# scientificcomputing/networks_fenicsx

Measured on NVIDIA B200. Metric: tree-network assemble+solve DOFs/s, higher is better.
Workload: dtype f64

## Files before the change

### networks_fenicsx_b200/_build.py

```python

from __future__ import annotations

import os
import pathlib
import shutil
import subprocess

CSRC = pathlib.Path(__file__).parent / "csrc"
LIB = CSRC / "libnxfx_b200.so"
SOURCES = ["nxfx_b200.cu"]
HEADERS = ["ctx.cuh", "assemble.cuh", "spmv.cuh", "precond.cuh", "generic.cuh", "condense.cuh", "peer.cuh", "../../include/nxfx_b200.h"]


def nvcc_path() -> str:
    for cand in (os.environ.get("NVCC"), shutil.which("nvcc"), "/usr/local/cuda/bin/nvcc"):
        if cand and os.path.exists(cand):
            return cand
    raise RuntimeError("nvcc not found; libnxfx_b200.so cannot be built")


def is_stale() -> bool:
    if not LIB.exists():
        return True
    t = LIB.stat().st_mtime
    return any((CSRC / f).resolve().stat().st_mtime > t for f in SOURCES + HEADERS)


def build_library(force: bool = False, verbose: bool = False) -> pathlib.Path:
    if not force and not is_stale():
        return LIB
    cmd = [
        nvcc_path(),
        "-gencode", "arch=compute_100a,code=sm_100a",
        "-O3", "-lineinfo", "-std=c++17",
        "-Xcompiler", "-fPIC", "-shared",
        "-o", str(LIB),
    ] + [str(CSRC / s) for s in SOURCES]
    if verbose:
        cmd.insert(1, "-Xptxas=-v")
    proc = subprocess.run(cmd, capture_output=True, text=True)
    if proc.returncode != 0:
        raise RuntimeError(f"nvcc failed:\n{' '.join(cmd)}\n{proc.stdout}\n{proc.stderr}")
    if verbose:
        print(proc.stderr)
    return LIB
```

### networks_fenicsx_b200/csrc/assemble.cuh

```cuda
#pragma once

#include "ctx.cuh"

namespace nxfx {

struct FastDiv {
  uint32_t magic, shift;
};
inline FastDiv make_fastdiv(uint32_t d) {
  FastDiv f;
  uint32_t fl = 31;
  while (!((d >> fl) & 1u)) --fl;
  if ((d & (d - 1)) == 0) {
    f.magic = 0;
    f.shift = fl == 0 ? 0 : fl - 1;
  } else {
    const uint64_t n = 1ull << (32 + fl);
    uint64_t m = n / d;
    const uint64_t rem = n % d;
    m += m;
    if (2 * rem >= d) m += 1;
    f.magic = (uint32_t)(m + 1);
    f.shift = fl;
  }
  return f;
}
__device__ __forceinline__ int fastdiv(int n, FastDiv f) {
  const uint32_t t = __umulhi((uint32_t)n, f.magic);
  return (int)(((((uint32_t)n - t) >> 1) + t) >> f.shift);
}

struct Net {
  int32_t n_nodes, E, N, n_bif;
  int32_t nq, poff, loff, ndofs;
  FastDiv div_np1, div_n;
  const int4* __restrict__ slot_uvl;
  const int32_t* __restrict__ slot_edge;
  const int32_t* __restrict__ edge_slot;
  const int32_t* __restrict__ bif_ptr;
  const int32_t* __restrict__ bif_inc;
  const double2* __restrict__ x2;
  const int2* __restrict__ slot_uv;
  const uint32_t* __restrict__ bif_in_bits;
};

constexpr unsigned int kLmTag = 0x7FF8B1F0u;
__device__ __forceinline__ double lm_box(int lm) {
  return __hiloint2double((int)kLmTag, lm);
}
__device__ __forceinline__ int lm_unbox(double p) {
  return (unsigned int)__double2hiint(p) == kLmTag ? __double2loint(p) : -1;
}

struct Coef {
  const double* __restrict__ R_cell;
  const double* __restrict__ f_cell;
  double R_const, f_const;
  double* __restrict__ cell_rh;
};

constexpr double kThird = 1.0 / 3.0;
constexpr double kSixth = 1.0 / 6.0;
constexpr int kMaxFluxRow = 7;

__device__ __forceinline__ int vertex_id(const Net& g, int e, int u, int v, int a) {
  return a == 0 ? u : (a == g.N ? v : g.n_nodes + e * (g.N - 1) + (a - 1));
}

struct VertexRec {
  double x, y, z, p;
};

__device__ __forceinline__ VertexRec load_vertex(const double2* __restrict__ x2, int v) {
  const double2* p = x2 + 2 * (size_t)v;
  const double2 a = __ldg(p), b = __ldg(p + 1);
  return VertexRec{a.x, a.y, b.x, b.y};
}

__device__ __forceinline__ double seg_length(const VertexRec& v0, const VertexRec& v1) {
  const double dx = __dsub_rn(v1.x, v0.x), dy = __dsub_rn(v1.y, v0.y), dz = __dsub_rn(v1.z, v0.z);
  return __dsqrt_rn(
      __dadd_rn(__dadd_rn(__dmul_rn(dx, dx), __dmul_rn(dy, dy)), __dmul_rn(dz, dz)));
}

__global__ void __launch_bounds__(kThreads)
pad_nodes_kernel(int n_nodes, int gdim, const double* __restrict__ pos, double* __restrict__ x) {
  int i = blockIdx.x * blockDim.x + threadIdx.x;
  if (i >= n_nodes * 3) return;
  int node = i / 3, d = i - node * 3;
  x[4 * (size_t)node + d] = d < gdim ? pos[(size_t)node * gdim + d] : 0.0;
}

__global__ void __launch_bounds__(kThreads)
set_pbc_kernel(int64_t nv, const double* __restrict__ pbc, double* __restrict__ x) {
  const int64_t i = blockIdx.x * (int64_t)blockDim.x + threadIdx.x;
  if (i < nv && lm_unbox(x[4 * i + 3]) < 0) x[4 * i + 3] = pbc[i];
}

__global__ void __launch_bounds__(kThreads)
tag_lm_kernel(int n_nodes, const int32_t* __restrict__ node_lm, double* __restrict__ x) {
  const int i = blockIdx.x * blockDim.x + threadIdx.x;
  if (i < n_nodes && node_lm[i] >= 0) x[4 * (size_t)i + 3] = lm_box(node_lm[i]);
}

__global__ void __launch_bounds__(kThreads)
interior_vertices_kernel(int n_nodes, int E, int N, const int32_t* __restrict__ eu,
                         const int32_t* __restrict__ ev, double* __restrict__ x) {
  const int64_t total = (int64_t)E * (N - 1) * 3;
  const double step = 1.0 / (double)N;
  for (int64_t i = blockIdx.x * (int64_t)blockDim.x + threadIdx.x; i < total;
       i += (int64_t)gridDim.x * blockDim.x) {
    const int64_t vert = i / 3;
    const int d = (int)(i - vert * 3);
    const int e = (int)(vert / (N - 1));
    const int k = (int)(vert - (int64_t)e * (N - 1)) + 1;
    const double w = __dmul_rn((double)k, step);
    const double s = x[4 * (size_t)eu[e] + d], t = x[4 * (size_t)ev[e] + d];
    x[4 * ((size_t)n_nodes + vert) + d] = __dadd_rn(__dmul_rn(s, __dsub_rn(1.0, w)), __dmul_rn(t, w));
  }
}

__device__ __forceinline__ int flux_row_cols(const Net& g, int r, int* cols) {
  const int N = g.N, np1 = N + 1;
  const int slot = r / np1, a = r - slot * np1;
  const int4 t = g.slot_uvl[slot];
  const int e = g.slot_edge[slot];
// ... 393 lines not shown
```

### networks_fenicsx_b200/csrc/ctx.cuh

```cuda
#pragma once

#include <cuda_runtime.h>

#include <cstdarg>
#include <cstdint>
#include <cstdio>
#include <cstring>
#include <string>
#include <vector>

#include "../../include/nxfx_b200.h"

namespace nxfx {

constexpr int kTileRows = 256;
constexpr int kTileCap = 2048;
constexpr int kThreads = 256;

template <typename T>
struct DevBuf {
  T* p = nullptr;
  size_t n = 0;
  cudaError_t alloc(size_t count) {
    release();
    n = count;
    if (count == 0) return cudaSuccess;
    return cudaMalloc(reinterpret_cast<void**>(&p), count * sizeof(T));
  }
  void release() {
    if (p) cudaFree(p);
    p = nullptr;
    n = 0;
  }
  ~DevBuf() { release(); }
};

struct TreeSchedule {
  bool set = false;
  int n_chunks = 0, n_lvl_ptr = 0, n_chords = 0, n_top = 0;
  int top_b0 = 0;
  std::vector<int32_t> t_of_bif_h;
  std::vector<int32_t> top_lvl_h;
  int sh_lmax = -1, pr_lmin = 0;
  int cap = 2048;
  DevBuf<int32_t> bif_of_t, chunk_desc, t_inc_ptr;
  DevBuf<int2> t_inc;
  DevBuf<double> lam_nat;
  DevBuf<int32_t> t_of_bif, t_parent, t_pedge, t_pslot, t_cptr, t_cidx, chunk_lptr, lvl_ptr, chord_edge;
  DevBuf<double> diag0, tg, d, gd, r, lam;
  bool fast_ok = false;
  bool coop_ok = false;
  bool coop_fs_ok = false;
  int coop_fs_blocks = 0;
  unsigned int epoch = 0;
};

struct MatState {
  int64_t id = 0;
  DevBuf<double> vals;
  DevBuf<double> cell_rh;
  bool assembled = false;
  int acc_count = 0;
};

struct Condensation {
  bool set = false;
  int n_max = 0, kl = 0, per_edge = 0, pcell_base = 0, pcell_stride = 0, cont = 0;
  DevBuf<int32_t> type_n, loc_ptr, loc_kind, loc_off, k_ptr, k_row, k_col, k_cell, c_ptr, c_row, c_slot, d_ptr, d_slot,
      d_col, bif_node, ipiv;
  DevBuf<double> k_coef, c_coef, d_coef, band, Y, S, y0, h, bd0, bU, bL, bDinv, bG, bH, br, bz;
  std::vector<int32_t> bif_node_h;
};

struct PeerComm {
  bool created = false, ready = false;
  bool in_process = false;
  bool shared_device = false;
  int rank = 0, nranks = 1;
  int slot = 0;
  void* local = nullptr;
  void* base[16] = {};
  unsigned int epoch[2] = {0, 0};
  int* err_h = nullptr;
  int* err_d = nullptr;
  DevBuf<double> lam_scratch;
};

}

struct nxfx_ctx {
  int device = 0;
  cudaStream_t stream = nullptr;
  std::string err;
  int64_t launches = 0;
  cudaEvent_t ev0 = nullptr, ev1 = nullptr;
  int sm_count = 148;

  bool has_network = false, has_pattern = false, has_pbc = false, pc_ready = false;
  bool bottom_factored = false;
  int32_t n_nodes = 0, E = 0, gdim = 0, N = 0, n_bif = 0, n_inc = 0;
  int64_t nv = 0, nc = 0, nq = 0, poff = 0, loff = 0, ndofs = 0, nnz = 0;
  nxfx::DevBuf<double> x;
  nxfx::DevBuf<double> pos_stage;
  nxfx::DevBuf<int4> slot_uvl;
  nxfx::DevBuf<int2> slot_uv;
  nxfx::DevBuf<uint32_t> bif_in_bits;
  nxfx::DevBuf<int32_t> slot_edge, edge_slot, edge_u, edge_v, bif_ptr, bif_inc;
  nxfx::DevBuf<int32_t> rowptr, colidx, tile_base;
  bool pipe_ok = false;
  bool generic = false;
  nxfx::DevBuf<int32_t> gen_src_id, gen_bptr, gen_bid;
  nxfx::DevBuf<double> gen_src_coef, gen_bcoef, gen_cell_h;
  nxfx::Condensation cond;
  std::vector<nxfx::MatState*> mats;
  nxfx::MatState* cur = nullptr;
  int64_t next_mat_id = 1;
  bool pc_unscaled = false;
  int64_t pc_mat = -1;
  std::vector<int32_t> edge_slot_h;
  nxfx::TreeSchedule tree;
  nxfx::DevBuf<double> edge_g, edge_c, edge_fn;
  nxfx::DevBuf<double> work;
  nxfx::DevBuf<double> work2;
  nxfx::DevBuf<double> scal;
  nxfx::DevBuf<unsigned int> ticket;
  double* scal_h = nullptr;
  double* scal_h_dev = nullptr;
  bool pdl_coop_refused = false;
  int32_t n_shared = 0;
  nxfx::DevBuf<int32_t> shared_lm;
  std::vector<int32_t> shared_lm_h;
  nxfx::DevBuf<int32_t> top_sh_pos;
  nxfx::DevBuf<int32_t> top_sh_idx;
  nxfx::DevBuf<double> lam_weight, lam_nonshared;
  nxfx::DevBuf<double> p_nonshared;
  nxfx::PeerComm comm;
  uint64_t peer_on = 0;
  double* mirror_h = nullptr;
  cudaStream_t side = nullptr;
  cudaEvent_t ev_x = nullptr;
  nxfx::DevBuf<double> e2e_pbc, e2e_b, e2e_x;
};

namespace nxfx {

inline int fail(nxfx_ctx* ctx, int code, const char* fmt, ...) {
  char buf[512];
  va_list ap;
  va_start(ap, fmt);
  vsnprintf(buf, sizeof buf, fmt, ap);
  va_end(ap);
  if (ctx) ctx->err = buf;
  return code;
}

#define NXFX_CUDA(ctx, call)                                                                  \
  do {                                                                                        \
    cudaError_t _e = (call);                                                                  \
    if (_e != cudaSuccess)                                                                    \
      return nxfx::fail(ctx, NXFX_ERR_CUDA, "%s:%d: %s -> %s", __FILE__, __LINE__, #call,     \
                        cudaGetErrorString(_e));                                              \
  } while (0)

#define NXFX_REQUIRE(ctx, cond, msg)                                                          \
  do {                                                                                        \
    if (!(cond)) return nxfx::fail(ctx, NXFX_ERR_INVALID, "%s: %s", __func__, msg);           \
  } while (0)

#define NXFX_LAUNCH(ctx, kernel, grid, block, smem, ...)                                      \
  do {                                                                                        \
    kernel<<<(grid), (block), (smem), (ctx)->stream>>>(__VA_ARGS__);                          \
    (ctx)->launches++;                                                                        \
    NXFX_CUDA(ctx, cudaGetLastError());                                                       \
  } while (0)

inline int64_t cdiv(int64_t a, int64_t b) { return (a + b - 1) / b; }

}
```

### networks_fenicsx_b200/csrc/nxfx_b200.cu

```cuda

#include <cub/device/device_scan.cuh>

#include <algorithm>
#include <atomic>
#include <chrono>
#include <cmath>
#include <cstdlib>

#include "assemble.cuh"
#include "ctx.cuh"
#include "condense.cuh"
#include "generic.cuh"
#include "precond.cuh"
#include "spmv.cuh"

using namespace nxfx;

namespace {

constexpr int kScalPartials = 8 * kMaxPartials;
constexpr int kScalSlots = 1024;

Net make_net(const nxfx_ctx* c) {
  Net g;
  g.n_nodes = c->n_nodes;
  g.E = c->E;
  g.N = c->N;
  g.n_bif = c->n_bif;
  g.nq = (int32_t)c->nq;
  g.poff = (int32_t)c->poff;
  g.loff = (int32_t)c->loff;
  g.ndofs = (int32_t)c->ndofs;
  g.div_np1 = make_fastdiv((uint32_t)c->N + 1);
  g.div_n = make_fastdiv((uint32_t)std::max(c->N, 2));
  g.slot_uvl = c->slot_uvl.p;
  g.slot_edge = c->slot_edge.p;
  g.edge_slot = c->edge_slot.p;
  g.bif_ptr = c->bif_ptr.p;
  g.bif_inc = c->bif_inc.p;
  g.x2 = reinterpret_cast<const double2*>(c->x.p);
  g.slot_uv = c->slot_uv.p;
  g.bif_in_bits = c->bif_in_bits.p;
  return g;
}

TreeDev make_tree(nxfx_ctx* c) {
  TreeDev t;
  auto& s = c->tree;
  t.t_of_bif = s.t_of_bif.p;
  t.bif_of_t = s.bif_of_t.p;
  t.chunk_desc = s.chunk_desc.p;
  t.t_inc_ptr = s.t_inc_ptr.p;
  t.t_inc = s.t_inc.p;
  t.lam_nat = s.lam_nat.p;
  t.cap = s.cap;
  t.top_sh_pos = c->top_sh_pos.p;
  t.n_sh = c->top_sh_pos.p ? c->n_shared : 0;
  t.sh_lmax = s.sh_lmax;
  t.pr_lmin = s.pr_lmin;
  t.t_parent = s.t_parent.p;
  t.t_pedge = s.t_pedge.p;
  t.t_pslot = s.t_pslot.p;
  t.t_cptr = s.t_cptr.p;
  t.t_cidx = s.t_cidx.p;
  t.chunk_lptr = s.chunk_lptr.p;
  t.lvl_ptr = s.lvl_ptr.p;
  t.diag0 = s.diag0.p;
  t.tg = s.tg.p;
  t.d = s.d.p;
  t.gd = s.gd.p;
  t.r = s.r.p;
  t.lam = s.lam.p;
  return t;
}

PeerDev make_peer(nxfx_ctx* c, int ch) {
  PeerDev p = {};
  if (!c->comm.ready) return p;
  for (int r = 0; r < c->comm.nranks; ++r) p.base[r] = reinterpret_cast<unsigned long long>(c->comm.base[r]);
  p.rank = c->comm.rank;
  p.nranks = c->comm.nranks;
  p.slot = c->comm.slot;
  p.epoch = ++c->comm.epoch[ch];
  p.err = c->comm.err_d;
  return p;
}

CondDev make_cond(nxfx_ctx* ctx) {
  auto& k = ctx->cond;
  CondDev c;
  c.n_max = k.n_max; c.kl = k.kl; c.kv = 2 * k.kl; c.ldab = 3 * k.kl + 1;
  c.per_edge = k.per_edge; c.pcell_base = k.pcell_base; c.pcell_stride = k.pcell_stride; c.cont = k.cont;
  c.type_n = k.type_n.p; c.loc_ptr = k.loc_ptr.p; c.loc_kind = k.loc_kind.p; c.loc_off = k.loc_off.p;
  c.k_ptr = k.k_ptr.p; c.k_row = k.k_row.p; c.k_col = k.k_col.p; c.k_cell = k.k_cell.p; c.k_coef = k.k_coef.p;
  c.c_ptr = k.c_ptr.p; c.c_row = k.c_row.p; c.c_slot = k.c_slot.p; c.c_coef = k.c_coef.p;
  c.d_ptr = k.d_ptr.p; c.d_slot = k.d_slot.p; c.d_col = k.d_col.p; c.d_coef = k.d_coef.p;
  c.bif_node = k.bif_node.p;
  c.band = k.band.p; c.ipiv = k.ipiv.p; c.Y = k.Y.p; c.S = k.S.p; c.y0 = k.y0.p; c.h = k.h.p;
  c.bd0 = k.bd0.p; c.bU = k.bU.p; c.bL = k.bL.p; c.bDinv = k.bDinv.p; c.bG = k.bG.p; c.bH = k.bH.p;
  c.br = k.br.p; c.bz = k.bz.p;
  return c;
}

int vec_grid(const nxfx_ctx* c, int64_t n) {
  return (int)std::max<int64_t>(1, std::min<int64_t>(cdiv(n, kThreads), (int64_t)c->sm_count * 8));
}

template <typename T>
int upload(nxfx_ctx* ctx, DevBuf<T>& buf, const T* src, size_t n) {
  NXFX_CUDA(ctx, buf.alloc(n));
  if (n) NXFX_CUDA(ctx, cudaMemcpyAsync(buf.p, src, n * sizeof(T), cudaMemcpyHostToDevice, ctx->stream));
  return NXFX_OK;
}

int update_top_shared(nxfx_ctx* ctx) {
  ctx->top_sh_pos.release();
  ctx->top_sh_idx.release();
  ctx->tree.sh_lmax = -1;
  ctx->tree.pr_lmin = 0;
  if (!ctx->tree.set || ctx->n_shared == 0 || ctx->tree.t_of_bif_h.empty()) return NXFX_OK;
  std::vector<int32_t> pos((size_t)ctx->n_shared);
  for (int32_t i = 0; i < ctx->n_shared; ++i) {
    const int32_t p = ctx->tree.t_of_bif_h[ctx->shared_lm_h[i]] - ctx->tree.top_b0;
    if (p < 0 || p >= ctx->tree.n_top)
      return fail(ctx, NXFX_ERR_INVALID, "shared multiplier %d is not in the top chunk of the schedule", ctx->shared_lm_h[i]);
// ... 46 lines not shown

void release_matrices(nxfx_ctx* ctx) {
  for (MatState* m : ctx->mats) delete m;
  ctx->mats.clear();
  ctx->cur = nullptr;
  ctx->pc_ready = false;
  ctx->pc_mat = -1;
}

int new_matrix(nxfx_ctx* ctx, int64_t id, MatState** out) {
  auto* m = new MatState();
  m->id = id;
  ctx->mats.push_back(m);
  NXFX_CUDA(ctx, m->vals.alloc((size_t)ctx->nnz + 8));
  NXFX_CUDA(ctx, cudaMemsetAsync(m->vals.p, 0, ((size_t)ctx->nnz + 8) * sizeof(double), ctx->stream));
  NXFX_CUDA(ctx, m->cell_rh.alloc((size_t)ctx->nc));
  NXFX_CUDA(ctx, cudaMemsetAsync(m->cell_rh.p, 0, (size_t)ctx->nc * sizeof(double), ctx->stream));
  if (out) *out = m;
  return NXFX_OK;
}

void note_lhs_assembled(nxfx_ctx* ctx, int accumulate) {
  MatState* m = ctx->cur;
  m->acc_count = (accumulate && m->assembled) ? m->acc_count + 1 : 1;
  m->assembled = true;
  ctx->pc_ready = false;
  ctx->bottom_factored = false;
}

void bind_matrix(nxfx_ctx* ctx, MatState* m) {
  if (ctx->cur != m) ctx->bottom_factored = false;
  ctx->cur = m;
  if (ctx->pc_ready && ctx->pc_mat != m->id) ctx->pc_ready = false;
}

void mark_factored(nxfx_ctx* ctx) {
  ctx->pc_ready = true;
  ctx->pc_mat = ctx->cur->id;
}

int ensure_matrix(nxfx_ctx* ctx) {
  if (ctx->cur) return NXFX_OK;
  for (MatState* m : ctx->mats)
    if (m->id == 0) { bind_matrix(ctx, m); return NXFX_OK; }
  MatState* m = nullptr;
  int rc = new_matrix(ctx, 0, &m);
  if (rc) return rc;
  bind_matrix(ctx, m);
  return NXFX_OK;
}

int build_vertices(nxfx_ctx* ctx) {
  const int n3 = ctx->n_nodes * 3;
  NXFX_LAUNCH(ctx, pad_nodes_kernel, (int)cdiv(n3, kThreads), kThreads, 0, ctx->n_nodes, ctx->gdim,
              ctx->pos_stage.p, ctx->x.p);
  if (ctx->N > 1) {
    const int64_t total = (int64_t)ctx->E * (ctx->N - 1) * 3;
    NXFX_LAUNCH(ctx, interior_vertices_kernel, vec_grid(ctx, total), kThreads, 0, ctx->n_nodes,
                ctx->E, ctx->N, ctx->edge_u.p, ctx->edge_v.p, ctx->x.p);
  }
  return NXFX_OK;
}

constexpr size_t kPipeSmem = kStages * sizeof(SpmvStage) + kStages * sizeof(uint64_t);
#ifndef NXFX_SPMV_BLOCKS
#define NXFX_SPMV_BLOCKS 5
#endif
constexpr int kPipeBlocksPerSM = NXFX_SPMV_BLOCKS;

int do_spmv(nxfx_ctx* ctx, const double* x, double* y) {
  const int ntiles = (int)cdiv(ctx->ndofs, kTileRows);
  if (ctx->pipe_ok) {
    const int grid = std::min(ntiles, ctx->sm_count * kPipeBlocksPerSM);
    NXFX_LAUNCH(ctx, spmv_pipe_kernel<0>, grid, kTileRows, kPipeSmem, (int)ctx->ndofs, ntiles,
                ctx->rowptr.p, ctx->colidx.p, ctx->cur->vals.p, ctx->tile_base.p, x, y, nullptr, nullptr,
                nullptr, nullptr);
    return NXFX_OK;
  }
  NXFX_LAUNCH(ctx, spmv_kernel<0>, ntiles, kTileRows, 0, (int)ctx->ndofs, ntiles, ctx->rowptr.p,
              ctx->colidx.p, ctx->cur->vals.p, x, y, nullptr, nullptr, nullptr, nullptr);
  return NXFX_OK;
}

int do_residual(nxfx_ctx* ctx, const double* b, const double* x, double* r, double* norm2_d, bool pdl = false) {
  const int ntiles = (int)cdiv(ctx->ndofs, kTileRows);
  if (ctx->comm.ready) {
    NXFX_REQUIRE(ctx, ctx->pipe_ok && ctx->lam_nonshared.p, "the fused partitioned residual needs the pipelined SpMV and nxfx_set_shared");
    const int grid = std::min(ntiles, ctx->sm_count * kPipeBlocksPerSM);
    cudaLaunchConfig_t cfg = {};
    cfg.gridDim = dim3(grid);
    cfg.blockDim = dim3(kTileRows);
    cfg.dynamicSmemBytes = kPipeSmem;
    cfg.stream = ctx->stream;
    cudaLaunchAttribute attr[1];
    attr[0].id = cudaLaunchAttributeProgrammaticStreamSerialization;
    attr[0].val.programmaticStreamSerializationAllowed = 1;
    cfg.attrs = attr;
    cfg.numAttrs = pdl ? 1 : 0;
    NXFX_CUDA(ctx, cudaLaunchKernelEx(&cfg, spmv_pipe_kernel<3>, (int)ctx->ndofs, ntiles, (const int32_t*)ctx->rowptr.p,
                                      (const int32_t*)ctx->colidx.p, (const double*)ctx->cur->vals.p,
                                      (const int32_t*)ctx->tile_base.p, x, r, b, ctx->scal.p, ctx->ticket.p, norm2_d,
                                      (int)ctx->loff, (const double*)ctx->lam_nonshared.p, (const double*)ctx->lam_weight.p,
                                      make_peer(ctx, 1), (const int32_t*)ctx->shared_lm.p, (int)ctx->n_shared,
                                      ctx->comm.lam_scratch.p));
    ctx->launches++;
    return NXFX_OK;
  }
  if (ctx->pipe_ok && !pdl) {
    const int grid = std::min(ntiles, ctx->sm_count * kPipeBlocksPerSM);
    NXFX_LAUNCH(ctx, spmv_pipe_kernel<1>, grid, kTileRows, kPipeSmem, (int)ctx->ndofs, ntiles,
                ctx->rowptr.p, ctx->colidx.p, ctx->cur->vals.p, ctx->tile_base.p, x, r, b, ctx->scal.p,
                ctx->ticket.p, norm2_d);
    return NXFX_OK;
  }
  if (ctx->pipe_ok) {
    const int grid = std::min(ntiles, ctx->sm_count * kPipeBlocksPerSM);
    cudaLaunchConfig_t cfg = {};
    cfg.gridDim = dim3(grid);
    cfg.blockDim = dim3(kTileRows);
    cfg.dynamicSmemBytes = kPipeSmem;
    cfg.stream = ctx->stream;
    cudaLaunchAttribute attr[1];
    attr[0].id = cudaLaunchAttributeProgrammaticStreamSerialization;
    attr[0].val.programmaticStreamSerializationAllowed = 1;
    cfg.attrs = attr;
    cfg.numAttrs = 1;
    NXFX_CUDA(ctx, cudaLaunchKernelEx(&cfg, spmv_pipe_kernel<1>, (int)ctx->ndofs, ntiles, (const int32_t*)ctx->rowptr.p,
                                      (const int32_t*)ctx->colidx.p, (const double*)ctx->cur->vals.p,
                                      (const int32_t*)ctx->tile_base.p, x, r, b, ctx->scal.p, ctx->ticket.p, norm2_d, 0,
                                      (const double*)nullptr, (const double*)nullptr, PeerDev{}, (const int32_t*)nullptr, 0,
                                      (double*)nullptr));
    ctx->launches++;
    return NXFX_OK;
  }
  const int grid = std::min(ntiles, kMaxPartials);
  NXFX_LAUNCH(ctx, spmv_kernel<1>, grid, kTileRows, 0, (int)ctx->ndofs, ntiles, ctx->rowptr.p,
              ctx->colidx.p, ctx->cur->vals.p, x, r, b, ctx->scal.p, ctx->ticket.p, norm2_d);
  return NXFX_OK;
}

template <int K>
int launch_multi_dot(nxfx_ctx* ctx, int n, const double* A, size_t stride, const double* w, double* out) {
  NXFX_LAUNCH(ctx, multi_dot_kernel<K>, vec_grid(ctx, n), kThreads, 0, n, A, stride, w, ctx->scal.p,
              ctx->ticket.p, out);
  return NXFX_OK;
}

int do_multi_dot(nxfx_ctx* ctx, int n, int k, const double* A, size_t stride, const double* w, double* out) {
  int j = 0;
  while (j < k) {
    const int m = std::min(8, k - j);
    const double* Aj = A + (size_t)j * stride;
    int rc = NXFX_OK;
    switch (m) {
      case 8: rc = launch_multi_dot<8>(ctx, n, Aj, stride, w, out + j); break;
      case 7: rc = launch_multi_dot<7>(ctx, n, Aj, stride, w, out + j); break;
      case 6: rc = launch_multi_dot<6>(ctx, n, Aj, stride, w, out + j); break;
      case 5: rc = launch_multi_dot<5>(ctx, n, Aj, stride, w, out + j); break;
      case 4: rc = launch_multi_dot<4>(ctx, n, Aj, stride, w, out + j); break;
      case 3: rc = launch_multi_dot<3>(ctx, n, Aj, stride, w, out + j); break;
      case 2: rc = launch_multi_dot<2>(ctx, n, Aj, stride, w, out + j); break;
      default: rc = launch_multi_dot<1>(ctx, n, Aj, stride, w, out + j); break;
    }
    if (rc) return rc;
    j += m;
  }
  return NXFX_OK;
// ... 669 lines not shown
  if (!ctx) return NXFX_ERR_INVALID;
  NXFX_CUDA(ctx, cudaMemcpyAsync(d, s, bytes, cudaMemcpyDeviceToHost, ctx->stream));
  return NXFX_OK;
}
int nxfx_memcpy_d2d(nxfx_ctx* ctx, void* d, const void* s, size_t bytes) {
  if (!ctx) return NXFX_ERR_INVALID;
  NXFX_CUDA(ctx, cudaMemcpyAsync(d, s, bytes, cudaMemcpyDeviceToDevice, ctx->stream));
  return NXFX_OK;
}
int nxfx_memset(nxfx_ctx* ctx, void* d, int byte, size_t bytes) {
  if (!ctx) return NXFX_ERR_INVALID;
  NXFX_CUDA(ctx, cudaMemsetAsync(d, byte, bytes, ctx->stream));
  return NXFX_OK;
}
int nxfx_timer_start(nxfx_ctx* ctx) {
  if (!ctx) return NXFX_ERR_INVALID;
  NXFX_CUDA(ctx, cudaEventRecord(ctx->ev0, ctx->stream));
  return NXFX_OK;
}
int nxfx_timer_stop(nxfx_ctx* ctx, double* ms) {
  if (!ctx || !ms) return NXFX_ERR_INVALID;
  NXFX_CUDA(ctx, cudaEventRecord(ctx->ev1, ctx->stream));
  NXFX_CUDA(ctx, cudaEventSynchronize(ctx->ev1));
  float f = 0.f;
  NXFX_CUDA(ctx, cudaEventElapsedTime(&f, ctx->ev0, ctx->ev1));
  *ms = f;
  return NXFX_OK;
}

int nxfx_set_network(nxfx_ctx* ctx, int32_t n_nodes, int32_t n_edges, int32_t gdim, int32_t N,
                     const double* node_pos, const int32_t* edge_u, const int32_t* edge_v,
                     const int32_t* edge_slot, const int32_t* node_lm, int32_t n_bif,
                     const int32_t* bif_ptr, const int32_t* bif_inc) {
  if (!ctx) return NXFX_ERR_INVALID;
  NXFX_REQUIRE(ctx, n_nodes > 0 && n_edges > 0 && N >= 1 && gdim >= 1 && gdim <= 3, "bad sizes");
  NXFX_REQUIRE(ctx, node_pos && edge_u && edge_v && edge_slot && node_lm && bif_ptr, "null input");
  NXFX_CUDA(ctx, cudaSetDevice(ctx->device));
  const int64_t E = n_edges;
  const int64_t nq = E * (N + 1), nc = E * N, ndofs = nq + nc + n_bif;
  const int64_t nv = (int64_t)n_nodes + E * (N - 1);
  NXFX_REQUIRE(ctx, ndofs < (int64_t)2147483000 && nv * 3 < (int64_t)2147483000, "network too large for int32 indexing");
  const int32_t n_inc = bif_ptr[n_bif];
  NXFX_REQUIRE(ctx, n_inc == 0 || bif_inc, "null incidence list");
  std::vector<int4> uvl((size_t)E);
  std::vector<int32_t> slot_edge((size_t)E, -1);
  for (int64_t e = 0; e < E; ++e) {
    const int32_t u = edge_u[e], v = edge_v[e], s = edge_slot[e];
    if (u < 0 || u >= n_nodes || v < 0 || v >= n_nodes || u == v)
      return fail(ctx, NXFX_ERR_INVALID, "edge %lld has invalid endpoints (%d, %d)", (long long)e, u, v);
    if (s < 0 || s >= E || slot_edge[s] != -1)
      return fail(ctx, NXFX_ERR_INVALID, "edge_slot is not a permutation (edge %lld -> %d)", (long long)e, s);
    if (node_lm[u] >= n_bif || node_lm[v] >= n_bif)
      return fail(ctx, NXFX_ERR_INVALID, "node_lm out of range at edge %lld", (long long)e);
    slot_edge[s] = (int32_t)e;
    uvl[s] = make_int4(u, v, node_lm[u], node_lm[v]);
  }
  for (int32_t k = 0; k < n_inc; ++k)
    if ((bif_inc[k] >> 1) < 0 || (bif_inc[k] >> 1) >= E)
      return fail(ctx, NXFX_ERR_INVALID, "bif_inc[%d] out of range", k);
  ctx->has_network = ctx->has_pattern = ctx->has_pbc = ctx->pc_ready = false;
  release_matrices(ctx);
  nxfx_comm_destroy(ctx);
  ctx->edge_slot_h.assign(edge_slot, edge_slot + E);
  ctx->n_shared = 0;
  ctx->shared_lm.release();
  ctx->shared_lm_h.clear();
  ctx->top_sh_pos.release();
  ctx->top_sh_idx.release();
  ctx->tree.t_of_bif_h.clear();
  ctx->lam_weight.release();
  ctx->lam_nonshared.release();
  ctx->p_nonshared.release();
  ctx->tree.set = false;
  ctx->n_nodes = n_nodes; ctx->E = n_edges; ctx->gdim = gdim; ctx->N = N; ctx->n_bif = n_bif;
  ctx->n_inc = n_inc; ctx->nv = nv; ctx->nc = nc; ctx->nq = nq; ctx->poff = nq; ctx->loff = nq + nc;
  ctx->ndofs = ndofs; ctx->nnz = 0;
  int rc;
  if ((rc = upload(ctx, ctx->pos_stage, node_pos, (size_t)n_nodes * gdim))) return rc;
  if ((rc = upload(ctx, ctx->edge_u, edge_u, (size_t)E))) return rc;
  if ((rc = upload(ctx, ctx->edge_v, edge_v, (size_t)E))) return rc;
  if ((rc = upload(ctx, ctx->edge_slot, edge_slot, (size_t)E))) return rc;
  if ((rc = upload(ctx, ctx->slot_edge, slot_edge.data(), (size_t)E))) return rc;
  if ((rc = upload(ctx, ctx->slot_uvl, uvl.data(), (size_t)E))) return rc;
  std::vector<int2> uv((size_t)E);
  for (int64_t s = 0; s < E; ++s) uv[s] = make_int2(uvl[s].x, uvl[s].y);
  if ((rc = upload(ctx, ctx->slot_uv, uv.data(), (size_t)E))) return rc;
  std::vector<uint32_t> in_bits((size_t)(n_inc + 31) / 32 + 1, 0u);
  for (int32_t k = 0; k < n_inc; ++k)
    if (bif_inc[k] & 1) in_bits[k >> 5] |= 1u << (k & 31);
  if ((rc = upload(ctx, ctx->bif_in_bits, in_bits.data(), in_bits.size()))) return rc;
  DevBuf<int32_t> node_lm_d;
  if ((rc = upload(ctx, node_lm_d, node_lm, (size_t)n_nodes))) return rc;
  if ((rc = upload(ctx, ctx->bif_ptr, bif_ptr, (size_t)n_bif + 1))) return rc;
  if ((rc = upload(ctx, ctx->bif_inc, bif_inc, (size_t)n_inc))) return rc;
  NXFX_CUDA(ctx, ctx->x.alloc((size_t)nv * 4));
  NXFX_CUDA(ctx, cudaMemsetAsync(ctx->x.p, 0, (size_t)nv * 4 * sizeof(double), ctx->stream));
  NXFX_CUDA(ctx, ctx->edge_g.alloc((size_t)E));
  NXFX_CUDA(ctx, ctx->edge_c.alloc((size_t)E));
  NXFX_CUDA(ctx, ctx->edge_fn.alloc((size_t)E));
  if ((rc = ensure_scal(ctx))) return rc;
  if ((rc = build_vertices(ctx))) return rc;
  NXFX_LAUNCH(ctx, tag_lm_kernel, (int)cdiv(n_nodes, kThreads), kThreads, 0, n_nodes, node_lm_d.p, ctx->x.p);
  NXFX_CUDA(ctx, cudaStreamSynchronize(ctx->stream));
  ctx->has_network = true;
  return NXFX_OK;
}

int nxfx_update_node_positions(nxfx_ctx* ctx, const double* node_pos) {
  if (!ctx) return NXFX_ERR_INVALID;
  NXFX_REQUIRE(ctx, ctx->has_network && node_pos, "no network / null input");
  NXFX_CUDA(ctx, cudaMemcpyAsync(ctx->pos_stage.p, node_pos, (size_t)ctx->n_nodes * ctx->gdim * sizeof(double),
                                 cudaMemcpyHostToDevice, ctx->stream));
  return build_vertices(ctx);
}

int nxfx_get_sizes(const nxfx_ctx* ctx, int64_t* nv, int64_t* nc, int64_t* ndofs, int64_t* nnz) {
  if (!ctx || !ctx->has_network) return NXFX_ERR_INVALID;
  if (nv) *nv = ctx->nv;
  if (nc) *nc = ctx->nc;
  if (ndofs) *ndofs = ctx->ndofs;
  if (nnz) *nnz = ctx->nnz;
  return NXFX_OK;
}

int nxfx_mesh_geometry_device(nxfx_ctx* ctx, const double** x) {
  if (!ctx || !x) return NXFX_ERR_INVALID;
  NXFX_REQUIRE(ctx, ctx->has_network, "no network");
  *x = ctx->x.p;
  return NXFX_OK;
}

int nxfx_symbolic(nxfx_ctx* ctx) {
  if (!ctx) return NXFX_ERR_INVALID;
  NXFX_REQUIRE(ctx, ctx->has_network, "no network");
  int rc;
  ctx->generic = false;
  const int n = (int)ctx->ndofs;
  Net g = make_net(ctx);
  DevBuf<int32_t> len;
  NXFX_CUDA(ctx, len.alloc((size_t)n + 1));
  NXFX_CUDA(ctx, ctx->rowptr.alloc((size_t)n + 1 + 8));
  NXFX_CUDA(ctx, cudaMemsetAsync(ctx->rowptr.p, 0, ((size_t)n + 9) * sizeof(int32_t), ctx->stream));
  NXFX_LAUNCH(ctx, row_len_kernel, (int)cdiv(n + 1, kThreads), kThreads, 0, g, len.p);
  size_t tmp_bytes = 0;
  NXFX_CUDA(ctx, cub::DeviceScan::ExclusiveSum(nullptr, tmp_bytes, len.p, ctx->rowptr.p, n + 1, ctx->stream));
  DevBuf<char> tmp;
  NXFX_CUDA(ctx, tmp.alloc(tmp_bytes));
  NXFX_CUDA(ctx, cub::DeviceScan::ExclusiveSum(tmp.p, tmp_bytes, len.p, ctx->rowptr.p, n + 1, ctx->stream));
  ctx->launches++;
  int32_t nnz = 0;
  NXFX_CUDA(ctx, cudaMemcpyAsync(&nnz, ctx->rowptr.p + n, sizeof(int32_t), cudaMemcpyDeviceToHost, ctx->stream));
  NXFX_CUDA(ctx, cudaStreamSynchronize(ctx->stream));
  NXFX_REQUIRE(ctx, nnz > 0, "pattern overflow (nnz does not fit int32)");
  ctx->nnz = nnz;
  NXFX_CUDA(ctx, ctx->colidx.alloc((size_t)nnz + 8));
  NXFX_CUDA(ctx, cudaMemsetAsync(ctx->colidx.p, 0, ((size_t)nnz + 8) * sizeof(int32_t), ctx->stream));
  NXFX_LAUNCH(ctx, fill_cols_kernel, (int)cdiv(n, kThreads), kThreads, 0, g, ctx->rowptr.p, ctx->colidx.p);
  if ((rc = setup_spmv_tiles(ctx))) return rc;
  release_matrices(ctx);
  ctx->has_pattern = true;
  return NXFX_OK;
}

int nxfx_matrix_create(nxfx_ctx* ctx, int64_t* mat_id) {
  if (!ctx || !mat_id) return NXFX_ERR_INVALID;
  NXFX_REQUIRE(ctx, ctx->has_pattern, "symbolic phase has not been run");
  MatState* m = nullptr;
  int rc = new_matrix(ctx, ctx->next_mat_id++, &m);
  if (rc) return rc;
  *mat_id = m->id;
  return NXFX_OK;
}

// ... 846 lines not shown
```

Baseline: 21.46 billion.

## Add structure-aware residual kernel for N=1 tree networks

Adds a specialized residual kernel for degree-1 (N=1) networks that exploits the known per-row structure: flux rows, pressure rows and Lagrange-multiplier rows are each handled by dedicated tile routines that compute column indices from slot/edge metadata instead of reading colidx. Matrix values are still streamed into shared memory via bulk async copies with mbarrier pipelining, and the residual and RHS norms are reduced in the same pass. This removes the colidx traffic and the indirect gathers of the generic CSR SpMV, at the cost of extra per-slot metadata buffers and a code path that relies on the exact CSR entry ordering.

New measurement: 21.82 billion (median of 6 runs). 1.7% higher.

```diff
diff --git a/networks_fenicsx_b200/_build.py b/networks_fenicsx_b200/_build.py
--- a/networks_fenicsx_b200/_build.py
+++ b/networks_fenicsx_b200/_build.py
@@ -9,7 +9,7 @@
 CSRC = pathlib.Path(__file__).parent / "csrc"
 LIB = CSRC / "libnxfx_b200.so"
 SOURCES = ["nxfx_b200.cu"]
-HEADERS = ["ctx.cuh", "assemble.cuh", "spmv.cuh", "precond.cuh", "generic.cuh", "condense.cuh", "peer.cuh", "../../include/nxfx_b200.h"]
+HEADERS = ["ctx.cuh", "assemble.cuh", "spmv.cuh", "precond.cuh", "generic.cuh", "condense.cuh", "peer.cuh", "residual_n1.cuh", "../../include/nxfx_b200.h"]
 
 
 def nvcc_path() -> str:
diff --git a/networks_fenicsx_b200/csrc/assemble.cuh b/networks_fenicsx_b200/csrc/assemble.cuh
--- a/networks_fenicsx_b200/csrc/assemble.cuh
+++ b/networks_fenicsx_b200/csrc/assemble.cuh
@@ -42,6 +42,8 @@
   const double2* __restrict__ x2;
   const int2* __restrict__ slot_uv;
   const uint32_t* __restrict__ bif_in_bits;
+  const int2* __restrict__ slot_lm;
+  const int32_t* __restrict__ inc_col;
 };
 
 constexpr unsigned int kLmTag = 0x7FF8B1F0u;
diff --git a/networks_fenicsx_b200/csrc/ctx.cuh b/networks_fenicsx_b200/csrc/ctx.cuh
--- a/networks_fenicsx_b200/csrc/ctx.cuh
+++ b/networks_fenicsx_b200/csrc/ctx.cuh
@@ -104,10 +104,13 @@
   nxfx::DevBuf<double> pos_stage;
   nxfx::DevBuf<int4> slot_uvl;
   nxfx::DevBuf<int2> slot_uv;
+  nxfx::DevBuf<int2> slot_lm;
+  nxfx::DevBuf<int32_t> inc_col;
   nxfx::DevBuf<uint32_t> bif_in_bits;
   nxfx::DevBuf<int32_t> slot_edge, edge_slot, edge_u, edge_v, bif_ptr, bif_inc;
   nxfx::DevBuf<int32_t> rowptr, colidx, tile_base;
   bool pipe_ok = false;
+  int res_n1_per_sm = 0;
   bool generic = false;
   nxfx::DevBuf<int32_t> gen_src_id, gen_bptr, gen_bid;
   nxfx::DevBuf<double> gen_src_coef, gen_bcoef, gen_cell_h;
diff --git a/networks_fenicsx_b200/csrc/nxfx_b200.cu b/networks_fenicsx_b200/csrc/nxfx_b200.cu
--- a/networks_fenicsx_b200/csrc/nxfx_b200.cu
+++ b/networks_fenicsx_b200/csrc/nxfx_b200.cu
@@ -12,6 +12,7 @@
 #include "condense.cuh"
 #include "generic.cuh"
 #include "precond.cuh"
+#include "residual_n1.cuh"
 #include "spmv.cuh"
 
 using namespace nxfx;
@@ -41,6 +42,8 @@
   g.x2 = reinterpret_cast<const double2*>(c->x.p);
   g.slot_uv = c->slot_uv.p;
   g.bif_in_bits = c->bif_in_bits.p;
+  g.slot_lm = c->slot_lm.p;
+  g.inc_col = c->inc_col.p;
   return g;
 }
 
@@ -253,7 +256,36 @@
   return NXFX_OK;
 }
 
+bool residual_n1_enabled() {
+  static const bool on = [] { const char* e = std::getenv("NXFX_RESIDUAL_N1"); return !(e && e[0] == '0'); }();
+  return on;
+}
+
+int residual_n1(nxfx_ctx* ctx, const double* b, const double* x, double* r, double* norm2_d, bool pdl) {
+  if (ctx->res_n1_per_sm == 0)
+    NXFX_CUDA(ctx, cudaOccupancyMaxActiveBlocksPerMultiprocessor(&ctx->res_n1_per_sm, residual_n1_kernel, kTileRows, kResSmem));
+  const int nft = (int)cdiv(ctx->E, kResFluxSlots), npt = (int)cdiv(ctx->E, kResPresRows);
+  const int ntiles = nft + npt + (int)cdiv(ctx->n_bif, kResLamRows);
+  cudaLaunchConfig_t cfg = {};
+  cfg.gridDim = dim3(std::min({ntiles, ctx->sm_count * std::max(ctx->res_n1_per_sm, 1), kMaxPartials}));
+  cfg.blockDim = dim3(kTileRows);
+  cfg.dynamicSmemBytes = kResSmem;
+  cfg.stream = ctx->stream;
+  cudaLaunchAttribute attr[1];
+  attr[0].id = cudaLaunchAttributeProgrammaticStreamSerialization;
+  attr[0].val.programmaticStreamSerializationAllowed = 1;
+  cfg.attrs = attr;
+  cfg.numAttrs = pdl ? 1 : 0;
+  NXFX_CUDA(ctx, cudaLaunchKernelEx(&cfg, residual_n1_kernel, make_net(ctx), (const int32_t*)ctx->rowptr.p,
+                                    (const double*)ctx->cur->vals.p, nft, npt, ntiles, x, r, b, ctx->scal.p,
+                                    ctx->ticket.p, norm2_d));
+  ctx->launches++;
+  return NXFX_OK;
+}
+
 int do_residual(nxfx_ctx* ctx, const double* b, const double* x, double* r, double* norm2_d, bool pdl = false) {
+  if (!ctx->generic && ctx->N == 1 && !ctx->comm.ready && residual_n1_enabled())
+    return residual_n1(ctx, b, x, r, norm2_d, pdl);
   const int ntiles = (int)cdiv(ctx->ndofs, kTileRows);
   if (ctx->comm.ready) {
     NXFX_REQUIRE(ctx, ctx->pipe_ok && ctx->lam_nonshared.p, "the fused partitioned residual needs the pipelined SpMV and nxfx_set_shared");
@@ -1089,13 +1121,20 @@
   if ((rc = upload(ctx, ctx->edge_slot, edge_slot, (size_t)E))) return rc;
   if ((rc = upload(ctx, ctx->slot_edge, slot_edge.data(), (size_t)E))) return rc;
   if ((rc = upload(ctx, ctx->slot_uvl, uvl.data(), (size_t)E))) return rc;
-  std::vector<int2> uv((size_t)E);
-  for (int64_t s = 0; s < E; ++s) uv[s] = make_int2(uvl[s].x, uvl[s].y);
+  std::vector<int2> uv((size_t)E), lm((size_t)E);
+  for (int64_t s = 0; s < E; ++s) {
+    uv[s] = make_int2(uvl[s].x, uvl[s].y);
+    lm[s] = make_int2(uvl[s].z, uvl[s].w);
+  }
   if ((rc = upload(ctx, ctx->slot_uv, uv.data(), (size_t)E))) return rc;
+  if ((rc = upload(ctx, ctx->slot_lm, lm.data(), (size_t)E))) return rc;
   std::vector<uint32_t> in_bits((size_t)(n_inc + 31) / 32 + 1, 0u);
   for (int32_t k = 0; k < n_inc; ++k)
     if (bif_inc[k] & 1) in_bits[k >> 5] |= 1u << (k & 31);
   if ((rc = upload(ctx, ctx->bif_in_bits, in_bits.data(), in_bits.size()))) return rc;
+  std::vector<int32_t> inc_col(N == 1 ? (size_t)n_inc : 0);
+  for (size_t k = 0; k < inc_col.size(); ++k) inc_col[k] = 2 * edge_slot[bif_inc[k] >> 1];
+  if ((rc = upload(ctx, ctx->inc_col, inc_col.data(), inc_col.size()))) return rc;
   DevBuf<int32_t> node_lm_d;
   if ((rc = upload(ctx, node_lm_d, node_lm, (size_t)n_nodes))) return rc;
   if ((rc = upload(ctx, ctx->bif_ptr, bif_ptr, (size_t)n_bif + 1))) return rc;
diff --git a/networks_fenicsx_b200/csrc/residual_n1.cuh b/networks_fenicsx_b200/csrc/residual_n1.cuh
--- /dev/null
+++ b/networks_fenicsx_b200/csrc/residual_n1.cuh
@@ -0,0 +1,230 @@
+#pragma once
+
+#include "assemble.cuh"
+#include "spmv.cuh"
+
+namespace nxfx {
+
+constexpr int kResFluxSlots = kTileRows;
+constexpr int kResPresRows = 4 * kTileRows;
+constexpr int kResLamRows = kTileRows;
+constexpr int kResCap = 10 * kResFluxSlots + 8;
+constexpr size_t kResSmem = kStages * (kResCap * sizeof(double) + sizeof(uint64_t));
+
+__device__ __forceinline__ void pdl_wait(bool first, const double*& x, const double*& b, double*& y) {
+  if (first) asm volatile("griddepcontrol.wait;" ::: "memory");
+  asm volatile("mov.b64 %0, %0;" : "+l"(x) :: "memory");
+  asm volatile("mov.b64 %0, %0;" : "+l"(b) :: "memory");
+  asm volatile("mov.b64 %0, %0;" : "+l"(y) :: "memory");
+}
+
+template <typename Wait>
+__device__ __forceinline__ void res_flux_tile(const Net& g, int tile, const double* V, const double* x,
+                                              const double* b, double* y, bool first,
+                                              const Wait& wait, int* warp_nl, double& nrm, double& nrb) {
+  const int tid = threadIdx.x, lane = tid & 31, w = tid >> 5;
+  const int slot = tile * kResFluxSlots + tid;
+  const bool active = slot < g.E;
+  int2 lm = make_int2(-1, -1);
+  int e = 0;
+  if (active) {
+    lm = __ldg(g.slot_lm + slot);
+    e = __ldg(g.slot_edge + slot);
+  }
+  const bool hu = lm.x >= 0, hv = lm.y >= 0;
+  const unsigned bu = __ballot_sync(0xffffffffu, hu), bv = __ballot_sync(0xffffffffu, hv);
+  const unsigned lt = (1u << lane) - 1u;
+  int pre = __popc(bu & lt) + __popc(bv & lt);
+  if (lane == 0) warp_nl[w] = __popc(bu) + __popc(bv);
+  __syncthreads();
+#pragma unroll
+  for (int k = 0; k < kTileRows / 32; ++k)
+    if (k < w) pre += warp_nl[k];
+  pdl_wait(first, x, b, y);
+  if (!active) {
+    wait();
+    return;
+  }
+  const int r = 2 * slot;
+  const double bu_ = __ldcs(b + r), bv_ = __ldcs(b + r + 1);
+  const double x0 = x[r], x1 = x[r + 1], xp = x[g.poff + e];
+  const double xu = hu ? x[g.loff + lm.x] : 0.0, xv = hv ? x[g.loff + lm.y] : 0.0;
+  const bool ufirst = !hv || (hu && lm.x < lm.y);
+  const double xl0 = ufirst ? xu : xv, xl1 = ufirst ? xv : xu;
+  const int nl = (int)hu + (int)hv;
+  wait();
+  const double* v0 = V + 6 * tid + 2 * pre;
+  const double* v1 = v0 + 3 + nl;
+  double a0 = 0.0, a1 = 0.0;
+  a0 = __dadd_rn(a0, __dmul_rn(v0[0], x0));
+  a1 = __dadd_rn(a1, __dmul_rn(v1[0], x0));
+  a0 = __dadd_rn(a0, __dmul_rn(v0[1], x1));
+  a1 = __dadd_rn(a1, __dmul_rn(v1[1], x1));
+  a0 = __dadd_rn(a0, __dmul_rn(v0[2], xp));
+  a1 = __dadd_rn(a1, __dmul_rn(v1[2], xp));
+  if (nl > 0) {
+    a0 = __dadd_rn(a0, __dmul_rn(v0[3], xl0));
+    a1 = __dadd_rn(a1, __dmul_rn(v1[3], xl0));
+  }
+  if (nl > 1) {
+    a0 = __dadd_rn(a0, __dmul_rn(v0[4], xl1));
+    a1 = __dadd_rn(a1, __dmul_rn(v1[4], xl1));
+  }
+  const double r0 = __dsub_rn(bu_, a0), r1 = __dsub_rn(bv_, a1);
+  if (y) {
+    y[r] = r0;
+    y[r + 1] = r1;
+  }
+  nrm += r0 * r0;
+  nrm += r1 * r1;
+  nrb += bu_ * bu_;
+  nrb += bv_ * bv_;
+}
+
+template <typename Wait>
+__device__ __forceinline__ void res_pres_tile(const Net& g, int tile, const double* V, const double* x,
+                                              const double* b, double* y, bool first,
+                                              const Wait& wait, double& nrm, double& nrb) {
+  constexpr int kPer = kResPresRows / kTileRows;
+  const int e0 = tile * kResPresRows;
+  int c[kPer];
+#pragma unroll
+  for (int j = 0; j < kPer; ++j) {
+    const int e = e0 + threadIdx.x + j * kTileRows;
+    c[j] = e < g.E ? 2 * __ldg(g.edge_slot + e) : -1;
+  }
+  pdl_wait(first, x, b, y);
+  double bi[kPer], xa[kPer], xb[kPer];
+#pragma unroll
+  for (int j = 0; j < kPer; ++j) {
+    if (c[j] >= 0) {
+      bi[j] = __ldcs(b + g.poff + e0 + threadIdx.x + j * kTileRows);
+      xa[j] = x[c[j]];
+      xb[j] = x[c[j] + 1];
+    }
+  }
+  wait();
+#pragma unroll
+  for (int j = 0; j < kPer; ++j) {
+    if (c[j] < 0) continue;
+    const int i = threadIdx.x + j * kTileRows;
+    double acc = 0.0;
+    acc = __dadd_rn(acc, __dmul_rn(V[2 * i], xa[j]));
+    acc = __dadd_rn(acc, __dmul_rn(V[2 * i + 1], xb[j]));
+    const double r = __dsub_rn(bi[j], acc);
+    if (y) y[g.poff + e0 + i] = r;
+    nrm += r * r;
+    nrb += bi[j] * bi[j];
+  }
+}
+
+__device__ __forceinline__ double res_lam_row(const Net& g, const double* V, int kt, int k0, int k1,
+                                              const double* __restrict__ x) {
+  double acc = 0.0;
+  for (int k = k0; k < k1; ++k) {
+    const int c0 = __ldg(g.inc_col + k);
+    acc = __dadd_rn(acc, __dmul_rn(V[2 * (k - kt)], x[c0]));
+    acc = __dadd_rn(acc, __dmul_rn(V[2 * (k - kt) + 1], x[c0 + 1]));
+  }
+  return acc;
+}
+
+template <typename Wait>
+__device__ __forceinline__ void res_lam_tile(const Net& g, int tile, const double* V, bool staged,
+                                             const double* __restrict__ vals, int sb, const double* x,
+                                             const double* b, double* y, bool first,
+                                             const Wait& wait, double& nrm, double& nrb) {
+  const int i0 = tile * kResLamRows, i = i0 + threadIdx.x;
+  const bool active = i < g.n_bif;
+  const int kt = __ldg(g.bif_ptr + i0);
+  int k0 = 0, k1 = 0;
+  if (active) {
+    k0 = __ldg(g.bif_ptr + i);
+    k1 = __ldg(g.bif_ptr + i + 1);
+  }
+  pdl_wait(first, x, b, y);
+  const double bi = active ? __ldcs(b + g.loff + i) : 0.0;
+  wait();
+  if (!active) return;
+  const double acc = staged ? res_lam_row(g, V, kt, k0, k1, x) : res_lam_row(g, vals + sb, kt, k0, k1, x);
+  const double r = __dsub_rn(bi, acc);
+  if (y) y[g.loff + i] = r;
+  nrm += r * r;
+  nrb += bi * bi;
+}
+
+__global__ void __launch_bounds__(kTileRows)
+residual_n1_kernel(Net g, const int32_t* __restrict__ rowptr, const double* __restrict__ vals, int nft, int npt,
+                   int ntiles, const double* __restrict__ x, double* __restrict__ y, const double* __restrict__ b,
+                   double* partial, unsigned int* ticket, double* norm2_out) {
+  extern __shared__ __align__(128) unsigned char smem_raw[];
+  double(*st)[kResCap] = reinterpret_cast<double(*)[kResCap]>(smem_raw);
+  uint64_t* full = reinterpret_cast<uint64_t*>(smem_raw + kStages * kResCap * sizeof(double));
+  __shared__ double red[kTileRows / 32];
+  __shared__ int warp_nl[kTileRows / 32];
+  const int tid = threadIdx.x;
+  if (tid == 0) {
+    for (int s = 0; s < kStages; ++s) mbar_init(full + s, 1);
+    asm volatile("fence.mbarrier_init.release.cluster;" ::: "memory");
+    asm volatile("fence.proxy.async.shared::cta;" ::: "memory");
+  }
+  __syncthreads();
+  const uint64_t stream_policy = l2_evict_first_policy();
+  auto rows = [&](int tile) {
+    if (tile < nft) {
+      const int r0 = tile * 2 * kResFluxSlots;
+      return make_int2(r0, min(r0 + 2 * kResFluxSlots, g.nq));
+    }
+    if (tile < nft + npt) {
+      const int r0 = g.poff + (tile - nft) * kResPresRows;
+      return make_int2(r0, min(r0 + kResPresRows, g.loff));
+    }
+    const int r0 = g.loff + (tile - nft - npt) * kResLamRows;
+    return make_int2(r0, min(r0 + kResLamRows, g.ndofs));
+  };
+  auto run_len = [](int sb, int se) {
+    const int cnt = ((se + 1) & ~1) - (sb & ~1);
+    return cnt <= kResCap ? cnt : 0;
+  };
+  auto issue = [&](int tile, int s) {
+    const int2 rr = rows(tile);
+    const int sb = __ldg(rowptr + rr.x), cnt = run_len(sb, __ldg(rowptr + rr.y));
+    mbar_expect_tx(full + s, (uint32_t)cnt * 8u);
+    if (cnt > 0) bulk_g2s_stream(st[s], vals + (sb & ~1), (uint32_t)cnt * 8u, full + s, stream_policy);
+  };
+  if (tid == 0) {
+    for (int k = 0; k < kStages - 1; ++k) {
+      const int tile = blockIdx.x + k * gridDim.x;
+      if (tile < ntiles) issue(tile, k);
+    }
+  }
+  double nrm = 0.0, nrb = 0.0;
+  int it = 0;
+  for (int tile = blockIdx.x; tile < ntiles; tile += gridDim.x, ++it) {
+    const int s = it % kStages;
+    if (tid == 0) {
+      const int pre = tile + (kStages - 1) * gridDim.x;
+      if (pre < ntiles) issue(pre, (it + kStages - 1) % kStages);
+    }
+    const int2 rr = rows(tile);
+    const int sb = __ldg(rowptr + rr.x);
+    const double* V = st[s] + (sb & 1);
+    const bool first = it == 0;
+    const uint32_t parity = (uint32_t)((it / kStages) & 1);
+    auto wait = [&] { mbar_wait(full + s, parity); };
+    if (tile < nft) {
+      res_flux_tile(g, tile, V, x, b, y, first, wait, warp_nl, nrm, nrb);
+    } else if (tile < nft + npt) {
+      res_pres_tile(g, tile - nft, V, x, b, y, first, wait, nrm, nrb);
+    } else {
+      const bool staged = run_len(sb, __ldg(rowptr + rr.y)) > 0;
+      res_lam_tile(g, tile - nft - npt, V, staged, vals, sb, x, b, y, first, wait, nrm, nrb);
+    }
+    asm volatile("fence.proxy.async.shared::cta;" ::: "memory");
+    __syncthreads();
+  }
+  double mine[2] = {block_sum<kTileRows>(nrm, red), block_sum<kTileRows>(nrb, red)};
+  finish_partials<kTileRows, 2>(mine, partial, gridDim.x, ticket, norm2_out, red);
+}
+
+}
```
